# openMVG/openMVG

Hardware: AMD Instinct MI355X
Metric: descriptor pairs/s (brute-force L2 2-NN + ratio matching) (higher is better)
Workload: dtype i8 (int32 accumulate); 1 GPU; 1000 images x 2000 SIFT-like uint8x128 descriptors, exhaustive pairs (499500 image pairs, 499500 on rank 0), ratio 0.8; parallelism=pair-sharded x1, no collective

## Files before the change

### openmvg_amd/csrc/mvgx_match.hip

```cpp
#include <hip/hip_runtime.h>

#include <algorithm>
#include <atomic>
#include <climits>
#include <condition_variable>
#include <cstdint>
#include <cstdlib>
#include <cstring>
#include <functional>
#include <mutex>
#include <string>
#include <thread>
#include <vector>

#include "mvgx_common.h"

namespace {

using mvgx::set_error;

typedef int v4i __attribute__((ext_vector_type(4)));
typedef int v16i __attribute__((ext_vector_type(16)));

constexpr int kDim = 128;
// ... 6 lines not shown
constexpr int kBlockQTiles = kWaves * kNQ;
constexpr int kRecQuads = 1 + kWaves;
constexpr int kStageBytes = kWinTiles * kTileBytes + kWinTiles * kTileRows * 4;
constexpr int kRPad = INT_MIN + 512;
constexpr int kCPad = -(1 << 27);
constexpr int kNegInit = -(1 << 28);
constexpr uint32_t kNoMatch = 0xFFFFFFFFu;
constexpr int kTailTiles = 16;

struct MatchParams {
  const int8_t* tiles;
  const int8_t* rows_slot;
  const int* rconst;
  const int* cinit;
  const int* qnorm;
  const uint32_t* perm;
  const uint32_t* rowpos;
  const uint8_t* rows_u8;
  const uint64_t* img_row_off;
  const uint32_t* img_tile_off;
  const uint32_t* img_n;
  const uint32_t* img_ntiles;
  const uint32_t* img_neven;
  const uint2* pairs;
  const uint2* work;
  const uint4* work8h;
  const uint4* work8;
  uint32_t n_work;
  uint32_t* best;
  int2* cd;
  uint32_t* count;
  uint32_t* errflag;
  uint32_t qstride;
  float ratio_sq;
};

__global__ __launch_bounds__(256) void row_norms_kernel(const uint8_t* __restrict__ rows,
                                                        const uint64_t* __restrict__ img_row_off,
                                                        const uint32_t* __restrict__ img_n, int* __restrict__ rownorm,
                                                        uint32_t* __restrict__ n_even) {
  const uint32_t img = blockIdx.y;
  const uint32_t n = img_n[img];
  const uint32_t r = blockIdx.x * blockDim.x + threadIdx.x;
  bool even = false;
  if (r < n) {
    const uint4* src = reinterpret_cast<const uint4*>(rows + (img_row_off[img] + r) * kDim);
// ... 60 lines not shown
}

__global__ __launch_bounds__(256) void build_tiles_kernel(const uint8_t* __restrict__ rows,
                                                          const uint64_t* __restrict__ img_row_off,
                                                          const uint32_t* __restrict__ img_tile_off,
                                                          const uint32_t* __restrict__ perm, int8_t* __restrict__ tiles,
                                                          int8_t* __restrict__ rows_slot) {
  const uint32_t img = blockIdx.y;
  const uint32_t ntiles_pad = img_tile_off[img + 1] - img_tile_off[img];
  const uint32_t t = blockIdx.x;
  if (t >= ntiles_pad) return;
  const uint32_t gt = img_tile_off[img] + t;
  const int c = threadIdx.x;
  const int s = c >> 6, lane = c & 63;
  const int m = lane & 31, h = lane >> 5;
  const uint32_t src_row = perm[(size_t)gt * kTileRows + m];
  uint4 v = make_uint4(0, 0, 0, 0);
  if (src_row != kNoMatch) {
    v = *reinterpret_cast<const uint4*>(rows + (img_row_off[img] + src_row) * kDim + (s * 2 + h) * 16);
    v.x ^= 0x80808080u; v.y ^= 0x80808080u; v.z ^= 0x80808080u; v.w ^= 0x80808080u;
  }
  *reinterpret_cast<uint4*>(tiles + (size_t)gt * kTileBytes + c * 16) = v;
  *reinterpret_cast<uint4*>(rows_slot + ((size_t)gt * kTileRows + m) * kDim + (s * 2 + h) * 16) = v;
}

__global__ __launch_bounds__(256) void fill_i32_kernel(int* __restrict__ p, size_t n, int value) {
  const size_t i = (size_t)blockIdx.x * blockDim.x + threadIdx.x;
  if (i < n) p[i] = value;
}

__device__ __forceinline__ int med3i(int a, int b, int c) { return max(min(a, b), min(max(a, b), c)); }

__device__ __forceinline__ uint32_t xcd_remap(uint32_t b, uint32_t nwg) {
  const uint32_t q = nwg >> 3, r = nwg & 7u;
  const uint32_t xcd = b & 7u, pos = b >> 3;
  const uint32_t base = (xcd < r) ? xcd * (q + 1) : r * (q + 1) + (xcd - r) * q;
  return base + pos;
}

enum StageMode { kStageRegs = 1, kStageGlds = 2, kStageGldsAsm = 3 };


__device__ __forceinline__ void glds16_asm(const void* gsrc, unsigned lds_dst) {
  unsigned keep;
  asm volatile(
      "s_mov_b32 %0, m0\n\ts_mov_b32 m0, %2\n\ts_nop 0\n\tglobal_load_lds_dwordx4 %1, off\n\ts_mov_b32 m0, %0"
// ... 425 lines not shown
      const int d0 = nq - W1, d1ub = nq - V2;
      const bool cand = valid && (__int2float_rn(d0) < __fmul_rn(p.ratio_sq, __int2float_rn(d1ub)));
      const size_t o = (size_t)wk.x * p.qstride + q;
      p.best[o] = cand ? ((uint32_t)s1 | ((uint32_t)hw << 3) | ((uint32_t)g1 << 4)) : kNoMatch;
      if (cand) p.cd[o] = make_int2(d0, d1ub);
    }
  }
}

constexpr int kNB16 = 2 * kNQ;
__global__ __launch_bounds__(256, 2) void l2_filter16_kernel(MatchParams p) {
  extern __shared__ __attribute__((aligned(16))) char smem[];

  const int lane = threadIdx.x & 63;
  const int wave = __builtin_amdgcn_readfirstlane(threadIdx.x >> 6);
  const int g4 = lane >> 4, par = g4 & 1;

  const uint32_t w = xcd_remap(blockIdx.x, gridDim.x);
  const uint4* rec = p.work8 + (size_t)kRecQuads * w;
  const uint4 wsh = rec[0], wun = rec[1 + wave];
  const uint32_t tileI0 = wsh.x;
  const int ntI = (int)wsh.y;
  const uint32_t pair = wun.x, tileJ0 = wun.y, qt0 = wun.z;
  const uint32_t ntJpad = wun.w;
  const int nwin = (ntI + kWinTiles - 1) / kWinTiles;

  const int lane_chunk = ((lane >> 5) * 64 + ((lane >> 4) & 1) * 32 + (lane & 15)) * 16;
  v4i b[kNB16][2];
  {
    const int8_t* qsrc = p.tiles + (size_t)(tileJ0 + qt0) * kTileBytes + lane_chunk;
#pragma unroll
    for (int n = 0; n < kNB16; ++n)
#pragma unroll
      for (int ks = 0; ks < 2; ++ks) b[n][ks] = *reinterpret_cast<const v4i*>(qsrc + (n >> 1) * kTileBytes + (n & 1) * 256 + ks * 2048);
  }

  const int8_t* gI = p.tiles + (size_t)tileI0 * kTileBytes;
  const int* gC = p.cinit + (size_t)tileI0 * kTileRows;

  uint32_t qperm[kNB16];
  int qn[kNB16];
#pragma unroll
  for (int n = 0; n < kNB16; ++n) {
    const bool inb = lane < 16 && qt0 + (uint32_t)(n >> 1) < ntJpad;
    const size_t qs = (size_t)tileJ0 * kTileRows + (qt0 + (uint32_t)(n >> 1)) * kTileRows + (uint32_t)(n & 1) * 16 + (uint32_t)(lane & 15);
    qperm[n] = inb ? p.perm[qs] : kNoMatch;
    qn[n] = inb ? p.qnorm[qs] : 0;
  }

  int TP[kNB16][4];
  int TW[kNB16][4];
  int Q1[kNB16], Q2[kNB16], Qg[kNB16];
#pragma unroll
  for (int n = 0; n < kNB16; ++n) {
#pragma unroll
    for (int c = 0; c < 4; ++c) { TP[n][c] = kNegInit; TW[n][c] = kNegInit; }
    Q1[n] = kNegInit; Q2[n] = kNegInit; Qg[n] = 0;
  }

  stage_window_glds_asm(smem, gI, gC, wave, lane);
#pragma unroll
  for (int n = 0; n < kNB16; ++n) {
#pragma unroll
    for (int ks = 0; ks < 2; ++ks) asm volatile("" : "+v"(b[n][ks]));
    asm volatile("" : "+v"(qperm[n]), "+v"(qn[n]));
  }

  for (int win = 0; win < nwin; ++win) {
    asm volatile("s_waitcnt vmcnt(0)" ::: "memory");
    __syncthreads();
    char* buf = smem + (win & 1) * kStageBytes;
    char* nbuf = smem + ((win + 1) & 1) * kStageBytes;
    if (win + 1 < nwin)
      stage_window_glds_asm(nbuf, gI + (size_t)(win + 1) * kWinTiles * kTileBytes, gC + (win + 1) * kWinRows, wave, lane);

    const int nt = min(kWinTiles, ntI - win * kWinTiles);
    const char* wb = buf + lane_chunk;
    const char* wc = buf + kWinTiles * kTileBytes + g4 * 16;
    v4i accA[4], accB[4];
#pragma unroll
    for (int i = 0; i < 4; ++i) accB[i] = v4i{kNegInit, kNegInit, kNegInit, kNegInit};

#define MVGX_GROUP16(ACC, N0, A, CV)                                                                       \
  _Pragma("unroll") for (int i_ = 0; i_ < 4; ++i_)                                                          \
    ACC[i_] = __builtin_amdgcn_mfma_i32_16x16x64_i8(A[0], b[(N0) + i_][0], CV, 0, 0, 0);                    \
  _Pragma("unroll") for (int i_ = 0; i_ < 4; ++i_)                                                          \
    ACC[i_] = __builtin_amdgcn_mfma_i32_16x16x64_i8(A[1], b[(N0) + i_][1], ACC[i_], 0, 0, 0);
#define MVGX_EPI16(ACC, N0, BLK)                                                                            \
// ... 49 lines not shown

#pragma unroll
  for (int n = 0; n < kNB16; ++n) {
    int p1 = kNegInit, p2 = kNegInit, pc = 0;
#pragma unroll
    for (int c = 0; c < 4; ++c) {
      const int v = TP[n][c];
      const bool better = v > p1;
      p2 = better ? p1 : max(p2, v);
      pc = better ? c : pc;
      p1 = better ? v : p1;
    }
    int W1 = 2 * p1 - par, V2 = max(2 * p2 - par, 2 * Q2[n] - par);
    int code = (4 * (pc >> 1) + 2 * (g4 >> 1) + (pc & 1)) | (par << 3) | (Qg[n] << 4);
#pragma unroll
    for (int x = 16; x <= 32; x <<= 1) {
      const int o1 = __shfl_xor(W1, x), o2 = __shfl_xor(V2, x), oc = __shfl_xor(code, x);
      const bool mine = W1 > o1;
      V2 = mine ? max(V2, o1) : max(o2, W1);
      code = mine ? code : oc;
      W1 = mine ? W1 : o1;
    }
    const uint32_t q = (qt0 + (uint32_t)(n >> 1)) * kTileRows + (uint32_t)(n & 1) * 16 + (uint32_t)(lane & 15);
    if (lane < 16 && qt0 + (uint32_t)(n >> 1) < ntJpad) {
      const bool valid = qperm[n] != kNoMatch;
      const int nq = qn[n];
      const int d0 = nq - W1, d1ub = nq - V2;
      const bool cand = valid && (__int2float_rn(d0) < __fmul_rn(p.ratio_sq, __int2float_rn(d1ub)));
      const size_t o = (size_t)pair * p.qstride + q;
      p.best[o] = cand ? (uint32_t)code : kNoMatch;
      if (cand) p.cd[o] = make_int2(d0, d1ub);
    }
  }
}

constexpr int kNQh = 2;
constexpr int kNBh = 2 * kNQh;
constexpr int kBlockQTilesH = kWaves * kNQh;
__global__ __launch_bounds__(256, 3) void l2_filter16h_kernel(MatchParams p) {
  extern __shared__ __attribute__((aligned(16))) char smem[];

  const int lane = threadIdx.x & 63;
  const int wave = __builtin_amdgcn_readfirstlane(threadIdx.x >> 6);
  const int g4 = lane >> 4, par = g4 & 1;

  const uint32_t w = xcd_remap(blockIdx.x, gridDim.x);
  const uint4 wr0 = p.work8h[2 * (size_t)w], wr1 = p.work8h[2 * (size_t)w + 1];
  const uint32_t pair = wr0.x;
  const uint32_t tileI0 = wr0.z, tileJ0 = wr0.w;
  const uint32_t ntJpad = wr1.y;
  const int ntI = (int)wr1.x;
// ... 124 lines not shown
      const int o1 = __shfl_xor(W1, x), o2 = __shfl_xor(V2, x), oc = __shfl_xor(code, x);
      const bool mine = W1 > o1;
      V2 = mine ? max(V2, o1) : max(o2, W1);
      code = mine ? code : oc;
      W1 = mine ? W1 : o1;
    }
    const uint32_t q = (qt0 + (uint32_t)(n >> 1)) * kTileRows + (uint32_t)(n & 1) * 16 + (uint32_t)(lane & 15);
    if (lane < 16 && qt0 + (uint32_t)(n >> 1) < ntJpad) {
      const bool valid = qperm[n] != kNoMatch;
      const int nq = qn[n];
      const int d0 = nq - W1, d1ub = nq - V2;
      const bool cand = valid && (__int2float_rn(d0) < __fmul_rn(p.ratio_sq, __int2float_rn(d1ub)));
      const size_t o = (size_t)pair * p.qstride + q;
      p.best[o] = cand ? (uint32_t)code : kNoMatch;
      if (cand) p.cd[o] = make_int2(d0, d1ub);
    }
  }
}

template <bool kWaveUnits>
__global__ __launch_bounds__(256) void l2_verify_kernel(MatchParams p) {
  const int lane = threadIdx.x & 63;
  const int wave = threadIdx.x >> 6;
  uint32_t pair, qt0, I, tileI0, tileJ0, ntJpad;
  if constexpr (kWaveUnits) {
    const uint4* rec = p.work8 + (size_t)kRecQuads * blockIdx.x;
    const uint4 wun = rec[1 + __builtin_amdgcn_readfirstlane(wave)];
    pair = wun.x; tileJ0 = wun.y; qt0 = wun.z; ntJpad = wun.w;
    tileI0 = rec[0].x;
    I = p.pairs[pair].x;
  } else {
    const uint2 wk = p.work[blockIdx.x];
    const uint2 ij = p.pairs[wk.x];
    pair = wk.x; qt0 = wk.y + (uint32_t)wave * kNQ;
    I = ij.x;
    tileI0 = p.img_tile_off[I]; tileJ0 = p.img_tile_off[ij.y];
    ntJpad = p.img_tile_off[ij.y + 1] - tileJ0;
  }
  const uint32_t nEvenI = p.img_neven[I], nOddI = p.img_n[I] - nEvenI;
  const int l16 = lane & 15, sub = lane >> 4;
  uint32_t accepted = 0;
  for (int part = 0; part < 2; ++part) {
    const uint32_t q0 = qt0 * kTileRows + (uint32_t)part * 64;
    const uint32_t q = q0 + lane;
    const bool inb = q < ntJpad * kTileRows;
    const uint32_t code = inb ? p.best[(size_t)pair * p.qstride + q] : kNoMatch;
    unsigned long long todo = __ballot(code != kNoMatch);
    while (todo) {
      unsigned long long m = todo;
      for (int i = 0; i < sub; ++i) m &= m - 1;
      const bool active = m != 0;
      const int src = active ? __builtin_ctzll(m) : 0;
      for (int i = 0; i < 4; ++i) todo &= todo - 1;
      const uint32_t cc = (uint32_t)__shfl((int)code, src);
      const uint32_t qs = q0 + (uint32_t)src;
      const int s1 = cc & 7, hw = (cc >> 3) & 1, g1 = (int)(cc >> 4);
      const int piece = l16 & 7, rsel = l16 >> 3;
      const int mrow = slot_row(2 * s1 + rsel, hw);
      const size_t slot0 = (size_t)tileI0 * kTileRows + (active ? (size_t)g1 * kWinTiles * kTileRows + mrow : 0);
      const size_t slotQ = (size_t)tileJ0 * kTileRows + (active ? qs : 0);
      const size_t o = (size_t)pair * p.qstride + (active ? qs : 0);
      const uint32_t tt = (uint32_t)g1 * kWinTiles + (uint32_t)piece;
      const size_t slotI = active ? slot0 + (size_t)piece * kTileRows : slot0;
      const bool valid = active && (tt * 16u + (uint32_t)(2 * s1 + rsel)) < (hw ? nOddI : nEvenI);
      int4 va[8];
#pragma unroll
      for (int c = 0; c < 8; ++c)
        va[c] = *reinterpret_cast<const int4*>(p.rows_slot + (slot0 + (active ? (size_t)c * kTileRows : 0)) * kDim + piece * 16);
      const int4 vb = *reinterpret_cast<const int4*>(p.rows_slot + slotQ * kDim + piece * 16);
      const int2 f = p.cd[o];
      const int f_d0 = f.x, f_d1 = f.y;
      int nb = __builtin_amdgcn_sdot4(vb.x, vb.x, 0, false);
      nb = __builtin_amdgcn_sdot4(vb.y, vb.y, nb, false);
      nb = __builtin_amdgcn_sdot4(vb.z, vb.z, nb, false);
      nb = __builtin_amdgcn_sdot4(vb.w, vb.w, nb, false);
      nb += __builtin_amdgcn_update_dpp(0, nb, 0xB1, 0xF, 0xF, true);
      nb += __builtin_amdgcn_update_dpp(0, nb, 0x4E, 0xF, 0xF, true);
      nb += __builtin_amdgcn_update_dpp(0, nb, 0x141, 0xF, 0xF, true);
      int dot = 0, na = 0;
#pragma unroll
      for (int c = 0; c < 8; ++c) {
        int part = __builtin_amdgcn_sdot4(va[c].x, vb.x, 0, false);
        part = __builtin_amdgcn_sdot4(va[c].y, vb.y, part, false);
        part = __builtin_amdgcn_sdot4(va[c].z, vb.z, part, false);
        part = __builtin_amdgcn_sdot4(va[c].w, vb.w, part, false);
        part += __builtin_amdgcn_update_dpp(0, part, 0xB1, 0xF, 0xF, true);
        part += __builtin_amdgcn_update_dpp(0, part, 0x4E, 0xF, 0xF, true);
        part += __builtin_amdgcn_update_dpp(0, part, 0x141, 0xF, 0xF, true);
        dot = (c == piece) ? part : dot;
        int sq = __builtin_amdgcn_sdot4(va[c].x, va[c].x, 0, false);
        sq = __builtin_amdgcn_sdot4(va[c].y, va[c].y, sq, false);
        sq = __builtin_amdgcn_sdot4(va[c].z, va[c].z, sq, false);
// ... 36 lines not shown
  uint32_t c = 0;
  const size_t base = (size_t)blockIdx.x * 16384;
  for (int k = 0; k < 64; ++k) {
    const size_t i = base + (size_t)k * 256 + threadIdx.x;
    if (i < n && best[i] != kNoMatch) ++c;
  }
  const unsigned long long m = __ballot(c != 0);
  (void)m;
  for (int off = 32; off > 0; off >>= 1) c += __shfl_down(c, off);
  if ((threadIdx.x & 63) == 0 && c) atomicAdd(&s_sum, c);
  __syncthreads();
  if (threadIdx.x == 0 && s_sum) atomicAdd(counter, s_sum);
}

__global__ __launch_bounds__(256) void count_candidates_units_kernel(MatchParams p, uint32_t* __restrict__ counter) {
  __shared__ uint32_t s_sum;
  if (threadIdx.x == 0) s_sum = 0;
  __syncthreads();
  const int lane = threadIdx.x & 63, wave = threadIdx.x >> 6;
  const uint4 wun = p.work8[(size_t)kRecQuads * blockIdx.x + 1 + wave];
  uint32_t c = 0;
  for (int part = 0; part < 2; ++part) {
    const uint32_t q = wun.z * kTileRows + (uint32_t)part * 64 + (uint32_t)lane;
    const bool cand = q < wun.w * kTileRows && p.best[(size_t)wun.x * p.qstride + q] != kNoMatch;
    c += (uint32_t)__popcll(__ballot(cand));
  }
  if (lane == 0 && c) atomicAdd(&s_sum, c);
  __syncthreads();
  if (threadIdx.x == 0 && s_sum) atomicAdd(counter, s_sum);
}

__global__ __launch_bounds__(256) void l2_top2_ratio_naive_kernel(MatchParams p) {
  const uint2 wk = p.work[blockIdx.x];
  const uint2 ij = p.pairs[wk.x];
  const uint32_t I = ij.x, J = ij.y;
  const uint32_t nI = p.img_n[I], nJ = p.img_n[J];
  const uint8_t* rowsI = p.rows_u8 + p.img_row_off[I] * kDim;
  const uint8_t* rowsJ = p.rows_u8 + p.img_row_off[J] * kDim;
  for (uint32_t q = wk.y * kTileRows + threadIdx.x; q < min(nJ, (wk.y + kBlockQTiles) * kTileRows);
       q += blockDim.x) {
    uint32_t qv[32];
#pragma unroll
    for (int k = 0; k < 32; ++k) qv[k] = reinterpret_cast<const uint32_t*>(rowsJ + (size_t)q * kDim)[k];
    int d0 = INT_MAX, d1 = INT_MAX;
    uint32_t i0 = 0;
    for (uint32_t i = 0; i < nI; ++i) {
      const uint32_t* dbr = reinterpret_cast<const uint32_t*>(rowsI + (size_t)i * kDim);
// ... 31 lines not shown
    s_part[threadIdx.x] += v;
    __syncthreads();
  }
  uint32_t run = s_part[threadIdx.x] - sum;
  for (uint32_t i = lo; i < hi; ++i) { offsets[i] = run; run += count[i]; }
  if (threadIdx.x == 1023) offsets[n] = s_part[1023];
}

__global__ __launch_bounds__(256) void compact_matches_kernel(const uint32_t* __restrict__ best,
                                                              const uint32_t* __restrict__ offsets,
                                                              const uint2* __restrict__ pairs,
                                                              const uint32_t* __restrict__ img_n,
                                                              const uint64_t* __restrict__ img_row_off,
                                                              const uint32_t* __restrict__ rowpos,
                                                              uint32_t n_pairs, uint32_t qstride,
                                                              uint2* __restrict__ out_ij) {
  const uint32_t pidx = blockIdx.x * 4 + (threadIdx.x >> 6);
  if (pidx >= n_pairs) return;
  const int lane = threadIdx.x & 63;
  const uint32_t off = offsets[pidx];
  if (offsets[pidx + 1] == off) return;
  const uint32_t J = pairs[pidx].y;
  const uint32_t nJ = img_n[J];
  const uint32_t* pos = rowpos + img_row_off[J];
  uint32_t run = off;
  for (uint32_t q0 = 0; q0 < nJ; q0 += 64) {
    const uint32_t q = q0 + lane;
    const uint32_t v = (q < nJ) ? best[(size_t)pidx * qstride + pos[q]] : kNoMatch;
    const bool ok = v != kNoMatch;
    const unsigned long long m = __ballot(ok);
    if (ok) {
      const uint32_t pre = (uint32_t)__popcll(m & ((1ull << lane) - 1ull));
      out_ij[run + pre] = make_uint2(v, q);
    }
    run += (uint32_t)__popcll(m);
  }
}

template <typename T>
struct DevBuf {
  T* p = nullptr;
  size_t cap = 0;
  int ensure(size_t n) {
    if (n <= cap) return MVGX_OK;
    if (p) { MVGX_HIP(hipFree(p)); p = nullptr; cap = 0; }
    const size_t want = std::max<size_t>(n, 16);
    MVGX_HIP(mvgx::device_malloc(reinterpret_cast<void**>(&p), want * sizeof(T)));
    cap = want;
    return MVGX_OK;
  }
  void release() { if (p) { (void)hipFree(p); p = nullptr; cap = 0; } }
// ... 37 lines not shown

}

struct mvgx_match_ctx {
  int device = 0;
  hipStream_t stream = nullptr;
  hipEvent_t ev_total0 = nullptr, ev_total1 = nullptr;
  int variant = 4;
  int filter_shape = 16;
  int stage = 3;
  int profile = 0;
  int64_t batch_pairs = 1 << 15;
  int keep_host_results = 1;
  int overlap = 1;
  int verify_alone = 0;
  int debug_filter = 0;
  int stream_hold = 0;
  int pinned_stream = 1;
  uint32_t n_images = 0;
  uint32_t total_tiles = 0;
  uint32_t max_tiles_pad = 0;
  uint32_t qstride = 0;
  std::vector<uint32_t> h_n, h_tile_off, h_ntiles;
  std::vector<uint64_t> h_row_off;
  DevBuf<uint8_t> d_rows;
  bool rows_owned = true;
  const uint8_t* d_rows_view = nullptr;
  DevBuf<int8_t> d_tiles, d_rows_slot;
  DevBuf<int> d_rconst, d_cinit, d_qnorm, d_rownorm;
  DevBuf<uint64_t> d_row_off;
  DevBuf<uint32_t> d_tile_off, d_n, d_ntiles, d_perm, d_rowpos, d_neven, d_err;
  struct Slot {
    hipStream_t stream = nullptr;
    hipEvent_t ev_scan = nullptr;
    hipEvent_t ev_filter = nullptr;
    DevBuf<uint2> d_pairs, d_work, d_ij;
    DevBuf<uint4> d_work8, d_work8h;
    DevBuf<uint32_t> d_best, d_count, d_offsets;
    DevBuf<int2> d_cd;
    PinnedBuf<uint2> hp_pairs, hp_work;
    PinnedBuf<uint4> hp_work8, hp_work8h;
    PinnedBuf<uint32_t> hp_offsets;
    uint64_t p0 = 0;
    uint32_t nb = 0;
    hipEvent_t ev_copy = nullptr;
    PinnedBuf<uint32_t> hp_ij[2];
    std::vector<uint32_t> h_off_out[2];
    int out_set = 0;
    uint64_t out_p0 = 0;
    uint32_t out_nb = 0;
  } slot[2];
  struct Results {
    std::vector<uint64_t> offsets;
    PinnedBuf<uint32_t> ij;
    size_t ij_n = 0;
  } results[2];
  int cur = 0;
  int double_buffer = 0;
  std::vector<hipEvent_t> ev_pool;
  std::vector<mvgx_match_ctx*> children;
};

namespace {

int prep_regions(mvgx_match_ctx* c) {
  const uint32_t n_images = c->n_images;
  c->h_tile_off.assign(n_images + 1, 0);
  c->h_row_off.assign(n_images + 1, 0);
  c->h_ntiles.assign(n_images + 1, 0);
  uint32_t max_n = 0;
  for (uint32_t k = 0; k < n_images; ++k) {
    c->h_row_off[k + 1] = c->h_row_off[k] + c->h_n[k];
    max_n = std::max(max_n, c->h_n[k]);
  }
  const uint64_t total_rows = c->h_row_off[n_images];
  int rc;
  if ((rc = c->d_row_off.ensure(n_images + 1))) return rc;
  if ((rc = c->d_tile_off.ensure(n_images + 1))) return rc;
  if ((rc = c->d_n.ensure(n_images + 1))) return rc;
  if ((rc = c->d_ntiles.ensure(n_images + 1))) return rc;
  if ((rc = c->d_neven.ensure(n_images + 1))) return rc;
  if ((rc = c->d_err.ensure(2))) return rc;
  if ((rc = c->d_rownorm.ensure(std::max<uint64_t>(total_rows, 1)))) return rc;
  if ((rc = c->d_rowpos.ensure(std::max<uint64_t>(total_rows, 1)))) return rc;
  MVGX_HIP(hipMemcpyAsync(c->d_row_off.p, c->h_row_off.data(), (n_images + 1) * sizeof(uint64_t),
                          hipMemcpyHostToDevice, c->stream));
  MVGX_HIP(hipMemcpyAsync(c->d_n.p, c->h_n.data(), n_images * sizeof(uint32_t), hipMemcpyHostToDevice, c->stream));
  MVGX_HIP(hipMemsetAsync(c->d_neven.p, 0, (n_images + 1) * sizeof(uint32_t), c->stream));
  MVGX_HIP(hipMemsetAsync(c->d_err.p, 0, 2 * sizeof(uint32_t), c->stream));
  std::vector<uint32_t> h_even(n_images + 1, 0);
  if (total_rows > 0) {
    dim3 grid((max_n + 255) / 256, n_images);
    hipLaunchKernelGGL(row_norms_kernel, grid, dim3(256), 0, c->stream, c->d_rows_view, c->d_row_off.p, c->d_n.p,
                       c->d_rownorm.p, c->d_neven.p);
    MVGX_HIP(hipGetLastError());
    MVGX_HIP(hipMemcpyAsync(h_even.data(), c->d_neven.p, n_images * sizeof(uint32_t), hipMemcpyDeviceToHost, c->stream));
  }
  MVGX_HIP(hipStreamSynchronize(c->stream));
  uint32_t max_pad = 0;
  for (uint32_t k = 0; k < n_images; ++k) {
    const uint32_t ne = h_even[k], no = c->h_n[k] - h_even[k];
    const uint32_t nt = (std::max(ne, no) + 15) / 16;
    const uint32_t pad = (nt + kWinTiles - 1) / kWinTiles * kWinTiles;
    c->h_ntiles[k] = nt;
    c->h_tile_off[k + 1] = c->h_tile_off[k] + pad;
    max_pad = std::max(max_pad, pad);
  }
  c->total_tiles = c->h_tile_off[n_images];
  c->max_tiles_pad = max_pad;
  c->qstride = max_pad * kTileRows;
  const size_t alloc_tiles = (size_t)c->total_tiles + kTailTiles;
  const size_t alloc_slots = alloc_tiles * kTileRows;
  if ((rc = c->d_tiles.ensure(alloc_tiles * kTileBytes))) return rc;
  if ((rc = c->d_rows_slot.ensure(alloc_tiles * kTileBytes))) return rc;
  if ((rc = c->d_rconst.ensure(alloc_slots))) return rc;
  if ((rc = c->d_cinit.ensure(alloc_slots))) return rc;
  if ((rc = c->d_qnorm.ensure(alloc_slots))) return rc;
  if ((rc = c->d_perm.ensure(alloc_slots))) return rc;
  MVGX_HIP(hipMemcpyAsync(c->d_tile_off.p, c->h_tile_off.data(), (n_images + 1) * sizeof(uint32_t),
                          hipMemcpyHostToDevice, c->stream));
  MVGX_HIP(hipMemcpyAsync(c->d_ntiles.p, c->h_ntiles.data(), (n_images + 1) * sizeof(uint32_t),
                          hipMemcpyHostToDevice, c->stream));
  const int fill_grid = (int)((alloc_slots + 255) / 256);
  hipLaunchKernelGGL(fill_i32_kernel, dim3(fill_grid), dim3(256), 0, c->stream, c->d_rconst.p, alloc_slots, kRPad);
  hipLaunchKernelGGL(fill_i32_kernel, dim3(fill_grid), dim3(256), 0, c->stream, c->d_cinit.p, alloc_slots, kCPad);
  hipLaunchKernelGGL(fill_i32_kernel, dim3(fill_grid), dim3(256), 0, c->stream, c->d_qnorm.p, alloc_slots, 0);
  hipLaunchKernelGGL(fill_i32_kernel, dim3(fill_grid), dim3(256), 0, c->stream, reinterpret_cast<int*>(c->d_perm.p),
                     alloc_slots, (int)kNoMatch);
  MVGX_HIP(hipGetLastError());
  MVGX_HIP(hipMemsetAsync(c->d_tiles.p + (size_t)c->total_tiles * kTileBytes, 0, (size_t)kTailTiles * kTileBytes,
                          c->stream));
  if (total_rows > 0 && max_pad > 0) {
    hipLaunchKernelGGL(assign_slots_kernel, dim3(n_images), dim3(1024), 0, c->stream, c->d_row_off.p, c->d_tile_off.p,
                       c->d_n.p, c->d_rownorm.p, c->d_rowpos.p, c->d_perm.p, c->d_rconst.p, c->d_cinit.p, c->d_qnorm.p);
    MVGX_HIP(hipGetLastError());
    dim3 grid(max_pad, n_images);
    hipLaunchKernelGGL(build_tiles_kernel, grid, dim3(256), 0, c->stream, c->d_rows_view, c->d_row_off.p,
                       c->d_tile_off.p, c->d_perm.p, c->d_tiles.p, c->d_rows_slot.p);
    MVGX_HIP(hipGetLastError());
  }
  MVGX_HIP(hipStreamSynchronize(c->stream));
  return MVGX_OK;
}

hipEvent_t get_event(mvgx_match_ctx* c, size_t i) {
  while (c->ev_pool.size() <= i) {
    hipEvent_t e = nullptr;
    if (hipEventCreate(&e) != hipSuccess) return nullptr;
    c->ev_pool.push_back(e);
  }
  return c->ev_pool[i];
}

}

extern "C" {

int mvgx_match_create_multi(const int* devices, int n_devices, mvgx_match_ctx** out) {
  MVGX_REQUIRE(out != nullptr && devices != nullptr && n_devices >= 1, MVGX_ERR_ARG, "mvgx_match_create_multi: bad argument");
  if (n_devices == 1) return mvgx_match_create(devices[0] < 0 ? -2 : devices[0], out);
  auto* c = new mvgx_match_ctx();
// ... 58 lines not shown
#else
    const bool ok = v == 0 || v == 8 || v == 16;
#endif
    if (ok) c->debug_filter = v;
    else fprintf(stderr, "[mvgx] MVGX_MATCH_FILTER=%s ignored (not a form this build of the library has)\n", e);
  }
  guard.c = nullptr;
  *out = c;
  return MVGX_OK;
}

int mvgx_match_destroy(mvgx_match_ctx* c) {
  if (!c) return MVGX_OK;
  if (!c->children.empty()) {
    for (mvgx_match_ctx* child : c->children) mvgx_match_destroy(child);
    for (auto& r : c->results) r.ij.release();
    delete c;
    return MVGX_OK;
  }
  (void)hipSetDevice(c->device);
  if (c->stream) (void)hipStreamSynchronize(c->stream);
  c->d_rows.release(); c->d_tiles.release(); c->d_rconst.release(); c->d_qnorm.release();
  c->d_rows_slot.release(); c->d_cinit.release(); c->d_rownorm.release(); c->d_ntiles.release(); c->d_perm.release(); c->d_rowpos.release();
  c->d_neven.release(); c->d_err.release();
  c->d_row_off.release(); c->d_tile_off.release(); c->d_n.release();
  for (auto& r : c->results) r.ij.release();
  for (auto& sl : c->slot) {
    sl.d_work8.release(); sl.hp_work8.release(); sl.d_work8h.release(); sl.hp_work8h.release();
    sl.d_pairs.release(); sl.d_work.release(); sl.d_ij.release(); sl.d_cd.release();
    sl.d_best.release(); sl.d_count.release(); sl.d_offsets.release();
    sl.hp_pairs.release(); sl.hp_work.release(); sl.hp_offsets.release(); sl.hp_ij[0].release(); sl.hp_ij[1].release();
    if (sl.ev_copy) (void)hipEventDestroy(sl.ev_copy);
    if (sl.ev_scan) (void)hipEventDestroy(sl.ev_scan);
    if (sl.ev_filter) (void)hipEventDestroy(sl.ev_filter);
    if (sl.stream) (void)hipStreamDestroy(sl.stream);
  }
  for (hipEvent_t e : c->ev_pool) (void)hipEventDestroy(e);
  if (c->ev_total0) (void)hipEventDestroy(c->ev_total0);
  if (c->ev_total1) (void)hipEventDestroy(c->ev_total1);
  if (c->stream) (void)hipStreamDestroy(c->stream);
  delete c;
  return MVGX_OK;
}

int mvgx_match_set_option(mvgx_match_ctx* c, const char* key, int64_t value) {
  MVGX_REQUIRE(c && key, MVGX_ERR_ARG, "mvgx_match_set_option: NULL argument");
  if (strcmp(key, "pinned_results") && strcmp(key, "double_buffer_results") && strcmp(key, "keep_host_results"))
// ... 126 lines not shown
  std::atomic<int> stop{0};
  bool take(uint64_t& p0, uint32_t& nb) {
    if (stop.load(std::memory_order_relaxed)) return false;
    p0 = next.fetch_add(B);
    if (p0 >= n_pairs) return false;
    nb = (uint32_t)std::min<uint64_t>(B, n_pairs - p0);
    return true;
  }
};

using BatchSink = std::function<int(uint64_t p0, uint32_t nb, const uint32_t* offsets, const uint32_t* ij)>;

int run_device(mvgx_match_ctx* c, BatchFeed& feed, float ratio_sq, const BatchSink* sink, mvgx_match_stats& st) {
  const uint32_t* pairs_IJ = feed.pairs_IJ;
  MVGX_HIP(hipSetDevice(c->device));
  mvgx_match_ctx::Results& res = c->results[c->cur];
  memset(&st, 0, sizeof(st));
  st.variant = (uint32_t)c->variant;
  size_t n_ev = 0;
  int rc;

  MVGX_HIP(hipEventRecord(c->ev_total0, c->slot[0].stream));

  auto issue = [&](mvgx_match_ctx::Slot& sl, mvgx_match_ctx::Slot* prev, uint64_t p0, uint32_t nb) -> int {
    int rc;
    hipStream_t stream = sl.stream;
    sl.p0 = p0; sl.nb = nb;
    if ((rc = sl.hp_pairs.ensure(nb))) return rc;
    const uint32_t max_blocks_per_pair = std::max<uint32_t>(1, (c->max_tiles_pad + kBlockQTiles - 1) / kBlockQTiles);
    if ((rc = sl.hp_work.ensure((size_t)nb * max_blocks_per_pair))) return rc;
    const bool records = c->variant == 4 && c->filter_shape == 16 && c->stage == 3 && !c->debug_filter;
    const bool records_h = c->variant == 4 && c->filter_shape == 17 && c->stage == 3 && !c->debug_filter;
    if (records && (rc = sl.hp_work8.ensure((size_t)nb * max_blocks_per_pair * kRecQuads))) return rc;
    if (records_h && (rc = sl.hp_work8h.ensure((size_t)nb * max_blocks_per_pair * 4))) return rc;
    uint32_t n_work_h = 0;
    uint32_t n_work = 0;
    uint32_t n_rec = 0, rec_used = kWaves, rec_I = 0;
    for (uint32_t k = 0; k < nb; ++k) {
      const uint32_t I = pairs_IJ[2 * (p0 + k)], J = pairs_IJ[2 * (p0 + k) + 1];
      sl.hp_pairs.p[k] = make_uint2(I, J);
      const uint32_t nI = c->h_n[I], nJ = c->h_n[J];
      if (nI < 2 || nJ == 0) continue;
      const uint32_t ntJ = c->h_ntiles[J];
      if (records)
        for (uint32_t qt = 0; qt < ntJ; qt += kNQ) {
          if (rec_used == kWaves || rec_I != I) {
            uint4* r = sl.hp_work8.p + (size_t)kRecQuads * n_rec++;
            r[0] = make_uint4(c->h_tile_off[I], c->h_ntiles[I], 0, 0);
            for (int w = 0; w < kWaves; ++w) r[1 + w] = make_uint4(0, c->h_tile_off[I], 0, 0);
            rec_used = 0; rec_I = I;
          }
          sl.hp_work8.p[(size_t)kRecQuads * (n_rec - 1) + 1 + rec_used++] = make_uint4(k, c->h_tile_off[J], qt, c->h_tile_off[J + 1] - c->h_tile_off[J]);
        }
      for (uint32_t qt = 0; qt < ntJ; qt += kBlockQTiles) {
        if (records_h)
          for (uint32_t q2 = qt; q2 < std::min(ntJ, qt + (uint32_t)kBlockQTiles); q2 += kBlockQTilesH) {
            sl.hp_work8h.p[2 * n_work_h] = make_uint4(k, q2, c->h_tile_off[I], c->h_tile_off[J]);
            sl.hp_work8h.p[2 * n_work_h + 1] = make_uint4(c->h_ntiles[I], c->h_tile_off[J + 1] - c->h_tile_off[J], 0, 0);
            ++n_work_h;
          }
        sl.hp_work.p[n_work++] = make_uint2(k, qt);
      }
      st.n_pairs += 1;
      st.n_desc_pairs += (uint64_t)nI * nJ;
    }
    if ((rc = sl.d_pairs.ensure(nb))) return rc;
    if ((rc = sl.d_work.ensure(std::max<uint32_t>(n_work, 1)))) return rc;
    if (records && (rc = sl.d_work8.ensure((size_t)std::max<uint32_t>(n_rec, 1) * kRecQuads))) return rc;
    if (records_h && (rc = sl.d_work8h.ensure((size_t)std::max<uint32_t>(n_work_h, 1) * 2))) return rc;
    if ((rc = sl.d_best.ensure((size_t)nb * c->qstride))) return rc;
    if (c->variant == 4) {
      if ((rc = sl.d_cd.ensure((size_t)nb * c->qstride))) return rc;
    }
    if ((rc = sl.d_count.ensure(nb))) return rc;
    if ((rc = sl.d_offsets.ensure((size_t)nb + 1))) return rc;
    if ((rc = sl.hp_offsets.ensure((size_t)nb + 1))) return rc;
    MVGX_HIP(hipMemcpyAsync(sl.d_pairs.p, sl.hp_pairs.p, nb * sizeof(uint2), hipMemcpyHostToDevice, stream));
    if (n_work && !records)
      MVGX_HIP(hipMemcpyAsync(sl.d_work.p, sl.hp_work.p, n_work * sizeof(uint2), hipMemcpyHostToDevice, stream));
    if (n_rec)
      MVGX_HIP(hipMemcpyAsync(sl.d_work8.p, sl.hp_work8.p, (size_t)n_rec * kRecQuads * sizeof(uint4), hipMemcpyHostToDevice, stream));
    if (n_work_h && records_h)
      MVGX_HIP(hipMemcpyAsync(sl.d_work8h.p, sl.hp_work8h.p, (size_t)n_work_h * 2 * sizeof(uint4), hipMemcpyHostToDevice, stream));
    MVGX_HIP(hipMemsetAsync(sl.d_count.p, 0, nb * sizeof(uint32_t), stream));

    MatchParams mp;
    mp.tiles = c->d_tiles.p; mp.rows_slot = c->d_rows_slot.p; mp.rconst = c->d_rconst.p; mp.cinit = c->d_cinit.p; mp.qnorm = c->d_qnorm.p;
    mp.perm = c->d_perm.p; mp.rowpos = c->d_rowpos.p;
    mp.rows_u8 = c->d_rows_view; mp.img_row_off = c->d_row_off.p;
    mp.img_tile_off = c->d_tile_off.p; mp.img_n = c->d_n.p; mp.img_ntiles = c->d_ntiles.p;
    mp.cd = sl.d_cd.p; mp.img_neven = c->d_neven.p; mp.errflag = c->d_err.p;
    mp.pairs = sl.d_pairs.p; mp.work = sl.d_work.p; mp.work8 = sl.d_work8.p; mp.work8h = sl.d_work8h.p; mp.n_work = n_work;
    mp.best = sl.d_best.p; mp.count = sl.d_count.p; mp.qstride = c->qstride; mp.ratio_sq = ratio_sq;

    if (prev) MVGX_HIP(hipStreamWaitEvent(stream, prev->ev_filter, 0));
    if (n_work) {
      hipEvent_t e0 = nullptr, e1 = nullptr;
      if (c->profile) {
        e0 = get_event(c, n_ev++); e1 = get_event(c, n_ev++);
        MVGX_REQUIRE(e0 && e1, MVGX_ERR_HIP, "hipEventCreate failed");
        MVGX_HIP(hipEventRecord(e0, stream));
      }
      if (c->variant == 0) {
        hipLaunchKernelGGL(l2_top2_ratio_naive_kernel, dim3(n_work), dim3(256), 0, stream, mp);
      } else if (c->variant == 1) {
        hipLaunchKernelGGL(l2_top2_ratio_kernel<kStageRegs>, dim3(n_work), dim3(256), 2 * kStageBytes, stream, mp);
      } else if (c->variant == 2) {
        hipLaunchKernelGGL(l2_top2_ratio_kernel<kStageGlds>, dim3(n_work), dim3(256), 2 * kStageBytes, stream, mp);
      } else if (c->variant == 3) {
        hipLaunchKernelGGL(l2_top2_ratio_kernel<kStageGldsAsm>, dim3(n_work), dim3(256), 2 * kStageBytes, stream, mp);
      } else if (c->filter_shape == 16 && c->stage == 3 && !c->debug_filter) {
// ... 41 lines not shown
    MVGX_HIP(hipGetLastError());
    MVGX_HIP(hipMemcpyAsync(sl.hp_offsets.p, sl.d_offsets.p, ((size_t)nb + 1) * sizeof(uint32_t), hipMemcpyDeviceToHost, stream));
    MVGX_HIP(hipEventRecord(sl.ev_scan, stream));
    return MVGX_OK;
  };
  auto finish = [&](mvgx_match_ctx::Slot& sl) -> int {
    int rc;
    MVGX_HIP(hipEventSynchronize(sl.ev_scan));
    const uint32_t nb = sl.nb;
    const uint64_t p0 = sl.p0;
    const uint32_t total = sl.hp_offsets.p[nb];
    if (sink) {
      if (c->stream_hold) sl.out_set ^= 1;
      sl.h_off_out[sl.out_set].assign(sl.hp_offsets.p, sl.hp_offsets.p + nb + 1);
    } else {
      const uint64_t base = res.offsets[p0];
      for (uint32_t k = 0; k <= nb; ++k) res.offsets[p0 + k] = base + sl.hp_offsets.p[k];
    }
    sl.out_p0 = p0; sl.out_nb = nb;
    st.n_matches += total;
    if (total) {
      if ((rc = sl.d_ij.ensure(total))) return rc;
      hipLaunchKernelGGL(compact_matches_kernel, dim3((nb + 3) / 4), dim3(256), 0, sl.stream, sl.d_best.p,
                         sl.d_offsets.p, sl.d_pairs.p, c->d_n.p, c->d_row_off.p, c->d_rowpos.p, nb, c->qstride,
                         sl.d_ij.p);
      MVGX_HIP(hipGetLastError());
      if (sink) {
        PinnedBuf<uint32_t>& hb = sl.hp_ij[sl.out_set];
        if (!hb.p) hb.pageable = !c->pinned_stream;
        if ((size_t)total * 2 > hb.cap) { hb.release(); if ((rc = hb.grow_keep(std::max<size_t>((size_t)total * 3, 4u << 20), 0))) return rc; }
        MVGX_HIP(hipMemcpyAsync(hb.p, sl.d_ij.p, (size_t)total * sizeof(uint2), hipMemcpyDeviceToHost, sl.stream));
      } else if (c->keep_host_results) {
        const size_t old = res.ij_n;
        if (old + (size_t)total * 2 > res.ij.cap)
          for (auto& o : c->slot) MVGX_HIP(hipStreamSynchronize(o.stream));
        if ((rc = res.ij.grow_keep(old + (size_t)total * 2, old))) return rc;
        res.ij_n = old + (size_t)total * 2;
        MVGX_HIP(hipMemcpyAsync(res.ij.p + old, sl.d_ij.p, (size_t)total * sizeof(uint2),
                                hipMemcpyDeviceToHost, sl.stream));
      }
    }
    if (sink) MVGX_HIP(hipEventRecord(sl.ev_copy, sl.stream));
    return MVGX_OK;
  };
  auto deliver = [&](mvgx_match_ctx::Slot& sl) -> int {
    MVGX_HIP(hipEventSynchronize(sl.ev_copy));
    if (feed.stop.load()) return MVGX_OK;
// ... 223 lines not shown
```

Baseline: 9726 billion descriptor pairs/s.

## Use dense unpermuted query tiles to skip padded query tiles in filter

Builds a separate dense query-side tile layout (rows in original order, tiles counted from the true image size) with its own norms, and drives the filter16 work records from it. Query tiles are no longer padded or permuted, so padded query tiles and the perm lookups and validity checks are dropped, and compaction indexes the best array directly. Verification now reads query rows straight from the raw u8 rows and flips the sign bit per load. The cost is extra device memory and a build kernel at setup, plus less regular query reads in verify.

```diff
diff --git a/openmvg_amd/csrc/mvgx_match.hip b/openmvg_amd/csrc/mvgx_match.hip
--- a/openmvg_amd/csrc/mvgx_match.hip
+++ b/openmvg_amd/csrc/mvgx_match.hip
@@ -52,6 +52,8 @@
   const uint32_t* img_n;
   const uint32_t* img_ntiles;
   const uint32_t* img_neven;
+  const int8_t* qtiles;
+  const int* qtnorm;
   const uint2* pairs;
   const uint2* work;
   const uint4* work8h;
@@ -158,6 +160,30 @@
   }
   *reinterpret_cast<uint4*>(tiles + (size_t)gt * kTileBytes + c * 16) = v;
   *reinterpret_cast<uint4*>(rows_slot + ((size_t)gt * kTileRows + m) * kDim + (s * 2 + h) * 16) = v;
+}
+
+__global__ __launch_bounds__(256) void build_qtiles_kernel(const uint8_t* __restrict__ rows,
+                                                           const uint64_t* __restrict__ img_row_off,
+                                                           const uint32_t* __restrict__ img_qtile_off,
+                                                           const uint32_t* __restrict__ img_n,
+                                                           const int* __restrict__ rownorm, int8_t* __restrict__ qtiles,
+                                                           int* __restrict__ qtnorm) {
+  const uint32_t img = blockIdx.y;
+  const uint32_t t = blockIdx.x;
+  if (t >= img_qtile_off[img + 1] - img_qtile_off[img]) return;
+  const uint32_t gt = img_qtile_off[img] + t;
+  const int c = threadIdx.x;
+  const int s = c >> 6, lane = c & 63;
+  const int m = lane & 31, h = lane >> 5;
+  const uint32_t r = t * kTileRows + (uint32_t)m;
+  const bool real = r < img_n[img];
+  uint4 v = make_uint4(0, 0, 0, 0);
+  if (real) {
+    v = *reinterpret_cast<const uint4*>(rows + (img_row_off[img] + r) * kDim + (s * 2 + h) * 16);
+    v.x ^= 0x80808080u; v.y ^= 0x80808080u; v.z ^= 0x80808080u; v.w ^= 0x80808080u;
+  }
+  *reinterpret_cast<uint4*>(qtiles + (size_t)gt * kTileBytes + c * 16) = v;
+  if (c < kTileRows) qtnorm[(size_t)gt * kTileRows + m] = real ? rownorm[img_row_off[img] + r] : 0;
 }
 
 __global__ __launch_bounds__(256) void fill_i32_kernel(int* __restrict__ p, size_t n, int value) {
@@ -629,13 +655,13 @@
   const uint32_t tileI0 = wsh.x;
   const int ntI = (int)wsh.y;
   const uint32_t pair = wun.x, tileJ0 = wun.y, qt0 = wun.z;
-  const uint32_t ntJpad = wun.w;
+  const uint32_t nJ = wun.w;
   const int nwin = (ntI + kWinTiles - 1) / kWinTiles;
 
   const int lane_chunk = ((lane >> 5) * 64 + ((lane >> 4) & 1) * 32 + (lane & 15)) * 16;
   v4i b[kNB16][2];
   {
-    const int8_t* qsrc = p.tiles + (size_t)(tileJ0 + qt0) * kTileBytes + lane_chunk;
+    const int8_t* qsrc = p.qtiles + (size_t)(tileJ0 + qt0) * kTileBytes + lane_chunk;
 #pragma unroll
     for (int n = 0; n < kNB16; ++n)
 #pragma unroll
@@ -645,14 +671,11 @@
   const int8_t* gI = p.tiles + (size_t)tileI0 * kTileBytes;
   const int* gC = p.cinit + (size_t)tileI0 * kTileRows;
 
-  uint32_t qperm[kNB16];
   int qn[kNB16];
 #pragma unroll
   for (int n = 0; n < kNB16; ++n) {
-    const bool inb = lane < 16 && qt0 + (uint32_t)(n >> 1) < ntJpad;
-    const size_t qs = (size_t)tileJ0 * kTileRows + (qt0 + (uint32_t)(n >> 1)) * kTileRows + (uint32_t)(n & 1) * 16 + (uint32_t)(lane & 15);
-    qperm[n] = inb ? p.perm[qs] : kNoMatch;
-    qn[n] = inb ? p.qnorm[qs] : 0;
+    const uint32_t q = (qt0 + (uint32_t)(n >> 1)) * kTileRows + (uint32_t)(n & 1) * 16 + (uint32_t)(lane & 15);
+    qn[n] = (lane < 16 && q < nJ) ? p.qtnorm[(size_t)tileJ0 * kTileRows + q] : 0;
   }
 
   int TP[kNB16][4];
@@ -670,7 +693,7 @@
   for (int n = 0; n < kNB16; ++n) {
 #pragma unroll
     for (int ks = 0; ks < 2; ++ks) asm volatile("" : "+v"(b[n][ks]));
-    asm volatile("" : "+v"(qperm[n]), "+v"(qn[n]));
+    asm volatile("" : "+v"(qn[n]));
   }
 
   for (int win = 0; win < nwin; ++win) {
@@ -766,11 +789,10 @@
       W1 = mine ? W1 : o1;
     }
     const uint32_t q = (qt0 + (uint32_t)(n >> 1)) * kTileRows + (uint32_t)(n & 1) * 16 + (uint32_t)(lane & 15);
-    if (lane < 16 && qt0 + (uint32_t)(n >> 1) < ntJpad) {
-      const bool valid = qperm[n] != kNoMatch;
+    if (lane < 16 && q < nJ) {
       const int nq = qn[n];
       const int d0 = nq - W1, d1ub = nq - V2;
-      const bool cand = valid && (__int2float_rn(d0) < __fmul_rn(p.ratio_sq, __int2float_rn(d1ub)));
+      const bool cand = __int2float_rn(d0) < __fmul_rn(p.ratio_sq, __int2float_rn(d1ub));
       const size_t o = (size_t)pair * p.qstride + q;
       p.best[o] = cand ? (uint32_t)code : kNoMatch;
       if (cand) p.cd[o] = make_int2(d0, d1ub);
@@ -941,20 +963,23 @@
 __global__ __launch_bounds__(256) void l2_verify_kernel(MatchParams p) {
   const int lane = threadIdx.x & 63;
   const int wave = threadIdx.x >> 6;
-  uint32_t pair, qt0, I, tileI0, tileJ0, ntJpad;
+  uint32_t pair, qt0, I, tileI0, tileJ0, qend;
+  const uint8_t* rowsJ = nullptr;
   if constexpr (kWaveUnits) {
     const uint4* rec = p.work8 + (size_t)kRecQuads * blockIdx.x;
     const uint4 wun = rec[1 + __builtin_amdgcn_readfirstlane(wave)];
-    pair = wun.x; tileJ0 = wun.y; qt0 = wun.z; ntJpad = wun.w;
+    pair = wun.x; tileJ0 = wun.y; qt0 = wun.z; qend = wun.w;
     tileI0 = rec[0].x;
-    I = p.pairs[pair].x;
+    const uint2 ij = p.pairs[pair];
+    I = ij.x;
+    rowsJ = p.rows_u8 + p.img_row_off[ij.y] * kDim;
   } else {
     const uint2 wk = p.work[blockIdx.x];
     const uint2 ij = p.pairs[wk.x];
     pair = wk.x; qt0 = wk.y + (uint32_t)wave * kNQ;
     I = ij.x;
     tileI0 = p.img_tile_off[I]; tileJ0 = p.img_tile_off[ij.y];
-    ntJpad = p.img_tile_off[ij.y + 1] - tileJ0;
+    qend = (p.img_tile_off[ij.y + 1] - tileJ0) * kTileRows;
   }
   const uint32_t nEvenI = p.img_neven[I], nOddI = p.img_n[I] - nEvenI;
   const int l16 = lane & 15, sub = lane >> 4;
@@ -962,7 +987,7 @@
   for (int part = 0; part < 2; ++part) {
     const uint32_t q0 = qt0 * kTileRows + (uint32_t)part * 64;
     const uint32_t q = q0 + lane;
-    const bool inb = q < ntJpad * kTileRows;
+    const bool inb = q < qend;
     const uint32_t code = inb ? p.best[(size_t)pair * p.qstride + q] : kNoMatch;
     unsigned long long todo = __ballot(code != kNoMatch);
     while (todo) {
@@ -986,7 +1011,13 @@
 #pragma unroll
       for (int c = 0; c < 8; ++c)
         va[c] = *reinterpret_cast<const int4*>(p.rows_slot + (slot0 + (active ? (size_t)c * kTileRows : 0)) * kDim + piece * 16);
-      const int4 vb = *reinterpret_cast<const int4*>(p.rows_slot + slotQ * kDim + piece * 16);
+      int4 vb;
+      if constexpr (kWaveUnits) {
+        vb = *reinterpret_cast<const int4*>(rowsJ + (size_t)(active ? qs : 0) * kDim + piece * 16);
+        vb.x ^= (int)0x80808080u; vb.y ^= (int)0x80808080u; vb.z ^= (int)0x80808080u; vb.w ^= (int)0x80808080u;
+      } else {
+        vb = *reinterpret_cast<const int4*>(p.rows_slot + slotQ * kDim + piece * 16);
+      }
       const int2 f = p.cd[o];
       const int f_d0 = f.x, f_d1 = f.y;
       int nb = __builtin_amdgcn_sdot4(vb.x, vb.x, 0, false);
@@ -1069,7 +1100,7 @@
   uint32_t c = 0;
   for (int part = 0; part < 2; ++part) {
     const uint32_t q = wun.z * kTileRows + (uint32_t)part * 64 + (uint32_t)lane;
-    const bool cand = q < wun.w * kTileRows && p.best[(size_t)wun.x * p.qstride + q] != kNoMatch;
+    const bool cand = q < wun.w && p.best[(size_t)wun.x * p.qstride + q] != kNoMatch;
     c += (uint32_t)__popcll(__ballot(cand));
   }
   if (lane == 0 && c) atomicAdd(&s_sum, c);
@@ -1147,11 +1178,11 @@
   if (offsets[pidx + 1] == off) return;
   const uint32_t J = pairs[pidx].y;
   const uint32_t nJ = img_n[J];
-  const uint32_t* pos = rowpos + img_row_off[J];
+  const uint32_t* pos = rowpos ? rowpos + img_row_off[J] : nullptr;
   uint32_t run = off;
   for (uint32_t q0 = 0; q0 < nJ; q0 += 64) {
     const uint32_t q = q0 + lane;
-    const uint32_t v = (q < nJ) ? best[(size_t)pidx * qstride + pos[q]] : kNoMatch;
+    const uint32_t v = (q < nJ) ? best[(size_t)pidx * qstride + (pos ? pos[q] : q)] : kNoMatch;
     const bool ok = v != kNoMatch;
     const unsigned long long m = __ballot(ok);
     if (ok) {
@@ -1235,14 +1266,15 @@
   uint32_t max_tiles_pad = 0;
   uint32_t qstride = 0;
   std::vector<uint32_t> h_n, h_tile_off, h_ntiles;
+  std::vector<uint32_t> h_qtile_off;
   std::vector<uint64_t> h_row_off;
   DevBuf<uint8_t> d_rows;
   bool rows_owned = true;
   const uint8_t* d_rows_view = nullptr;
-  DevBuf<int8_t> d_tiles, d_rows_slot;
-  DevBuf<int> d_rconst, d_cinit, d_qnorm, d_rownorm;
+  DevBuf<int8_t> d_tiles, d_rows_slot, d_qtiles;
+  DevBuf<int> d_rconst, d_cinit, d_qnorm, d_rownorm, d_qtnorm;
   DevBuf<uint64_t> d_row_off;
-  DevBuf<uint32_t> d_tile_off, d_n, d_ntiles, d_perm, d_rowpos, d_neven, d_err;
+  DevBuf<uint32_t> d_tile_off, d_qtile_off, d_n, d_ntiles, d_perm, d_rowpos, d_neven, d_err;
   struct Slot {
     hipStream_t stream = nullptr;
     hipEvent_t ev_scan = nullptr;
@@ -1281,15 +1313,18 @@
   c->h_tile_off.assign(n_images + 1, 0);
   c->h_row_off.assign(n_images + 1, 0);
   c->h_ntiles.assign(n_images + 1, 0);
+  c->h_qtile_off.assign(n_images + 1, 0);
   uint32_t max_n = 0;
   for (uint32_t k = 0; k < n_images; ++k) {
     c->h_row_off[k + 1] = c->h_row_off[k] + c->h_n[k];
+    c->h_qtile_off[k + 1] = c->h_qtile_off[k] + (c->h_n[k] + kTileRows - 1) / kTileRows;
     max_n = std::max(max_n, c->h_n[k]);
   }
   const uint64_t total_rows = c->h_row_off[n_images];
   int rc;
   if ((rc = c->d_row_off.ensure(n_images + 1))) return rc;
   if ((rc = c->d_tile_off.ensure(n_images + 1))) return rc;
+  if ((rc = c->d_qtile_off.ensure(n_images + 1))) return rc;
   if ((rc = c->d_n.ensure(n_images + 1))) return rc;
   if ((rc = c->d_ntiles.ensure(n_images + 1))) return rc;
   if ((rc = c->d_neven.ensure(n_images + 1))) return rc;
@@ -1330,6 +1365,12 @@
   if ((rc = c->d_cinit.ensure(alloc_slots))) return rc;
   if ((rc = c->d_qnorm.ensure(alloc_slots))) return rc;
   if ((rc = c->d_perm.ensure(alloc_slots))) return rc;
+  const size_t total_qtiles = c->h_qtile_off[n_images];
+  if ((rc = c->d_qtiles.ensure((total_qtiles + kTailTiles) * kTileBytes))) return rc;
+  if ((rc = c->d_qtnorm.ensure((total_qtiles + kTailTiles) * kTileRows))) return rc;
+  MVGX_HIP(hipMemcpyAsync(c->d_qtile_off.p, c->h_qtile_off.data(), (n_images + 1) * sizeof(uint32_t), hipMemcpyHostToDevice, c->stream));
+  MVGX_HIP(hipMemsetAsync(c->d_qtiles.p + total_qtiles * kTileBytes, 0, (size_t)kTailTiles * kTileBytes, c->stream));
+  MVGX_HIP(hipMemsetAsync(c->d_qtnorm.p + total_qtiles * kTileRows, 0, (size_t)kTailTiles * kTileRows * sizeof(int), c->stream));
   MVGX_HIP(hipMemcpyAsync(c->d_tile_off.p, c->h_tile_off.data(), (n_images + 1) * sizeof(uint32_t),
                           hipMemcpyHostToDevice, c->stream));
   MVGX_HIP(hipMemcpyAsync(c->d_ntiles.p, c->h_ntiles.data(), (n_images + 1) * sizeof(uint32_t),
@@ -1350,6 +1391,10 @@
     dim3 grid(max_pad, n_images);
     hipLaunchKernelGGL(build_tiles_kernel, grid, dim3(256), 0, c->stream, c->d_rows_view, c->d_row_off.p,
                        c->d_tile_off.p, c->d_perm.p, c->d_tiles.p, c->d_rows_slot.p);
+    MVGX_HIP(hipGetLastError());
+    dim3 qgrid((max_n + kTileRows - 1) / kTileRows, n_images);
+    hipLaunchKernelGGL(build_qtiles_kernel, qgrid, dim3(256), 0, c->stream, c->d_rows_view, c->d_row_off.p, c->d_qtile_off.p, c->d_n.p,
+                       c->d_rownorm.p, c->d_qtiles.p, c->d_qtnorm.p);
     MVGX_HIP(hipGetLastError());
   }
   MVGX_HIP(hipStreamSynchronize(c->stream));
@@ -1454,7 +1499,7 @@
   if (c->stream) (void)hipStreamSynchronize(c->stream);
   c->d_rows.release(); c->d_tiles.release(); c->d_rconst.release(); c->d_qnorm.release();
   c->d_rows_slot.release(); c->d_cinit.release(); c->d_rownorm.release(); c->d_ntiles.release(); c->d_perm.release(); c->d_rowpos.release();
-  c->d_neven.release(); c->d_err.release();
+  c->d_neven.release(); c->d_err.release(); c->d_qtiles.release(); c->d_qtnorm.release(); c->d_qtile_off.release();
   c->d_row_off.release(); c->d_tile_off.release(); c->d_n.release();
   for (auto& r : c->results) r.ij.release();
   for (auto& sl : c->slot) {
@@ -1627,6 +1672,7 @@
 
   MVGX_HIP(hipEventRecord(c->ev_total0, c->slot[0].stream));
 
+  const bool dense_queries = c->variant == 4 && c->filter_shape == 16 && c->stage == 3 && !c->debug_filter;
   auto issue = [&](mvgx_match_ctx::Slot& sl, mvgx_match_ctx::Slot* prev, uint64_t p0, uint32_t nb) -> int {
     int rc;
     hipStream_t stream = sl.stream;
@@ -1634,7 +1680,7 @@
     if ((rc = sl.hp_pairs.ensure(nb))) return rc;
     const uint32_t max_blocks_per_pair = std::max<uint32_t>(1, (c->max_tiles_pad + kBlockQTiles - 1) / kBlockQTiles);
     if ((rc = sl.hp_work.ensure((size_t)nb * max_blocks_per_pair))) return rc;
-    const bool records = c->variant == 4 && c->filter_shape == 16 && c->stage == 3 && !c->debug_filter;
+    const bool records = dense_queries;
     const bool records_h = c->variant == 4 && c->filter_shape == 17 && c->stage == 3 && !c->debug_filter;
     if (records && (rc = sl.hp_work8.ensure((size_t)nb * max_blocks_per_pair * kRecQuads))) return rc;
     if (records_h && (rc = sl.hp_work8h.ensure((size_t)nb * max_blocks_per_pair * 4))) return rc;
@@ -1647,15 +1693,16 @@
       const uint32_t nI = c->h_n[I], nJ = c->h_n[J];
       if (nI < 2 || nJ == 0) continue;
       const uint32_t ntJ = c->h_ntiles[J];
+      const uint32_t ntJq = c->h_qtile_off[J + 1] - c->h_qtile_off[J];
       if (records)
-        for (uint32_t qt = 0; qt < ntJ; qt += kNQ) {
+        for (uint32_t qt = 0; qt < ntJq; qt += kNQ) {
           if (rec_used == kWaves || rec_I != I) {
             uint4* r = sl.hp_work8.p + (size_t)kRecQuads * n_rec++;
             r[0] = make_uint4(c->h_tile_off[I], c->h_ntiles[I], 0, 0);
-            for (int w = 0; w < kWaves; ++w) r[1 + w] = make_uint4(0, c->h_tile_off[I], 0, 0);
+            for (int w = 0; w < kWaves; ++w) r[1 + w] = make_uint4(0, c->h_qtile_off[I], 0, 0);
             rec_used = 0; rec_I = I;
           }
-          sl.hp_work8.p[(size_t)kRecQuads * (n_rec - 1) + 1 + rec_used++] = make_uint4(k, c->h_tile_off[J], qt, c->h_tile_off[J + 1] - c->h_tile_off[J]);
+          sl.hp_work8.p[(size_t)kRecQuads * (n_rec - 1) + 1 + rec_used++] = make_uint4(k, c->h_qtile_off[J], qt, nJ);
         }
       for (uint32_t qt = 0; qt < ntJ; qt += kBlockQTiles) {
         if (records_h)
@@ -1691,7 +1738,7 @@
 
     MatchParams mp;
     mp.tiles = c->d_tiles.p; mp.rows_slot = c->d_rows_slot.p; mp.rconst = c->d_rconst.p; mp.cinit = c->d_cinit.p; mp.qnorm = c->d_qnorm.p;
-    mp.perm = c->d_perm.p; mp.rowpos = c->d_rowpos.p;
+    mp.perm = c->d_perm.p; mp.rowpos = c->d_rowpos.p; mp.qtiles = c->d_qtiles.p; mp.qtnorm = c->d_qtnorm.p;
     mp.rows_u8 = c->d_rows_view; mp.img_row_off = c->d_row_off.p;
     mp.img_tile_off = c->d_tile_off.p; mp.img_n = c->d_n.p; mp.img_ntiles = c->d_ntiles.p;
     mp.cd = sl.d_cd.p; mp.img_neven = c->d_neven.p; mp.errflag = c->d_err.p;
@@ -1779,7 +1826,7 @@
     if (total) {
       if ((rc = sl.d_ij.ensure(total))) return rc;
       hipLaunchKernelGGL(compact_matches_kernel, dim3((nb + 3) / 4), dim3(256), 0, sl.stream, sl.d_best.p,
-                         sl.d_offsets.p, sl.d_pairs.p, c->d_n.p, c->d_row_off.p, c->d_rowpos.p, nb, c->qstride,
+                         sl.d_offsets.p, sl.d_pairs.p, c->d_n.p, c->d_row_off.p, dense_queries ? nullptr : c->d_rowpos.p, nb, c->qstride,
                          sl.d_ij.p);
       MVGX_HIP(hipGetLastError());
       if (sink) {
```

Result: faster. 9943 billion descriptor pairs/s (median of 6 runs) (+2.2%).
